# aperezhortal/pySPEEDY

Measured on AMD Instinct MI355X. Metric: simulated-years/day (whole node), T30L8, higher is better.
Workload: dtype f64

## Files before the change

### include/pyspeedy_amd.h

```cpp
#ifndef PYSPEEDY_AMD_H
#define PYSPEEDY_AMD_H

#include <stddef.h>
#include <stdint.h>

#ifdef __cplusplus
extern "C" {
#endif

#define SPD_IX 96
#define SPD_IL 48
#define SPD_IY 24
#define SPD_KX 8
#define SPD_MX 31
#define SPD_NX 32
#define SPD_TRUNC 30

#define SPD_OK 0
#define SPD_E_ARG (-1)
#define SPD_E_DEVICE (-2)
#define SPD_E_SIZE (-3)
#define SPD_E_TIMEOUT (-4)

typedef struct spd_context *spd_handle;

int spd_create(spd_handle *out, int device);
int spd_destroy(spd_handle h);
int spd_device(spd_handle h);
const char *spd_last_error(void);
const char *spd_version(void);

long spd_get_table_host(spd_handle h, const char *name, double *buf_host, size_t buf_elems);

int spd_calendar_walk(int year, int month, int day, int hour, int minute, int nsteps, int32_t *ymdhm, int32_t *month_idx,
                      int32_t *imont1, double *tmonth, double *tyear);
int spd_daily_forcing_host(double tyear, double *out);

int spd_spec2grid(spd_handle h, const double *spec, double *grid, int kcos, int nfields, void *stream);
int spd_grid2spec(spd_handle h, const double *grid, double *spec, int nfields, void *stream);
int spd_legendre_inv(spd_handle h, const double *spec, double *four, int nfields, void *stream);
int spd_legendre(spd_handle h, const double *four, double *spec, int nfields, void *stream);
int spd_fourier_inv(spd_handle h, const double *four, double *grid, int kcos, int nfields, void *stream);
int spd_fourier(spd_handle h, const double *grid, double *four, int nfields, void *stream);

int spd_vort2vel(spd_handle h, const double *vor, const double *div, double *ucos, double *vcos, int nfields,
                 void *stream);
int spd_vel2vort(spd_handle h, const double *ucos, const double *vcos, double *vor, double *div, int nfields,
                 void *stream);
int spd_grid_vel2vort(spd_handle h, const double *ug, const double *vg, double *vor, double *div, int kcos,
                      int nfields, void *stream);
int spd_gradient(spd_handle h, const double *psi, double *psdx, double *psdy, int nfields, void *stream);
int spd_laplacian(spd_handle h, const double *in, double *out, int inverse, int nfields, void *stream);
int spd_truncate(spd_handle h, double *field, int nfields, void *stream);
int spd_grid_filter(spd_handle h, const double *fg1, double *fg2, int nfields, void *stream);

typedef struct spd_physics_args {
    const double *ug, *vg, *tg, *qg, *phig;
    const double *pslg;
    double *utend, *vtend, *ttend, *qtend;
    const double *fmask_land, *phis0, *forog, *sst_am, *alb_land, *alb_sea, *snowc, *land_temp, *soil_avail_water;
    const double *flux_solar_in, *flux_ozone_upper, *flux_ozone_lower, *zenit_correction, *stratospheric_correction,
        *alb_surface;
    double *precnv, *precls, *cbmf, *slrd, *slr, *olr;
    double *slru, *ustr, *vstr, *shf, *evap, *hfluxn;
    double *rad_st4a;
    double *rad_flux;
    double *tt_rsw;
    double *rad_tau2;
    double *rad_strat_corr;
    double *tsr, *ssrd, *ssr, *qcloud_equiv;
    int32_t *iptop, *icltop;
    double *ts, *tskin, *u0, *v0, *t0, *cloudc, *clstr;
// ... 125 lines not shown
```

### pyspeedy_amd/_lib.py

```python
import ctypes as C
import os
import subprocess

_HERE = os.path.dirname(os.path.abspath(__file__))
LIB_PATH = os.environ.get("PYSPEEDY_AMD_LIB") or os.path.join(_HERE, "libpyspeedy_amd.so")
CSRC = os.path.join(_HERE, "csrc")

IX, IL, IY, KX, MX, NX, TRUNC = 96, 48, 24, 8, 31, 32, 30
NSPEC, NFOUR, NGRID = MX * NX, 2 * MX * IL, IX * IL

SPD_OK, SPD_E_ARG, SPD_E_DEVICE, SPD_E_SIZE = 0, -1, -2, -3
SPD_STATS_MEAN, SPD_STATS_VARIANCE, SPD_STATS_STD = 0, 1, 2


class SpeedyHipError(RuntimeError):
    pass


def build(verbose=False):
    cmd = ["make", "-C", CSRC, "-j4"]
    if not verbose:
        cmd.insert(1, "-s")
    subprocess.run(cmd, check=True)
    if not os.path.isfile(LIB_PATH):
# ... 16 lines not shown
    _fields_ = [(n, C.c_void_p) for n in _PHYS_PTR_FIELDS] + [
        ("air_absortivity_co2", C.c_double), ("compute_shortwave", C.c_int32), ("fp32", C.c_int32),
        ("sppt_pattern", C.c_void_p)]


class ModelControl(C.Structure):
    _fields_ = [(n, C.c_int32) for n in (
        "current_step", "year", "month", "day", "hour", "minute", "month_idx", "land_coupling_flag",
        "sst_anomaly_coupling_flag", "increase_co2", "sppt_on", "sppt_first", "physics_fp32", "reserved")] + [
        ("sppt_step", C.c_int64), ("sppt_first_member_id", C.c_int64), ("sppt_seed", C.c_uint64),
        ("air_absortivity_co2", C.c_double), ("ablco2_ref", C.c_double)]


class StreamProbeArgs(C.Structure):
    _fields_ = [(n, C.c_int32) for n in (
        "reads", "writes", "lane_bytes", "in_flight", "nontemporal", "waves_per_simd", "rows_per_wave", "reps", "layout",
        "reserved")] + [
        ("total_bytes", C.c_uint64)]


_SIGNATURES = {
    "spd_stream_probe": (C.c_int, [C.c_void_p, C.POINTER(StreamProbeArgs), C.POINTER(C.c_double), C.POINTER(C.c_double),
                                   C.POINTER(C.c_uint64), C.POINTER(C.c_uint64)]),
    "spd_create": (C.c_int, [C.POINTER(C.c_void_p), C.c_int]),
    "spd_destroy": (C.c_int, [C.c_void_p]),
    "spd_device": (C.c_int, [C.c_void_p]),
    "spd_last_error": (C.c_char_p, []),
    "spd_version": (C.c_char_p, []),
    "spd_get_table_host": (C.c_long, [C.c_void_p, C.c_char_p, C.c_void_p, C.c_size_t]),
    "spd_calendar_walk": (C.c_int, [C.c_int] * 6 + [C.c_void_p] * 5),
    "spd_daily_forcing_host": (C.c_int, [C.c_double, C.c_void_p]),
    "spd_spec2grid": (C.c_int, [C.c_void_p, C.c_void_p, C.c_void_p, C.c_int, C.c_int, C.c_void_p]),
    "spd_grid2spec": (C.c_int, [C.c_void_p, C.c_void_p, C.c_void_p, C.c_int, C.c_void_p]),
    "spd_legendre_inv": (C.c_int, [C.c_void_p, C.c_void_p, C.c_void_p, C.c_int, C.c_void_p]),
    "spd_legendre": (C.c_int, [C.c_void_p, C.c_void_p, C.c_void_p, C.c_int, C.c_void_p]),
    "spd_fourier_inv": (C.c_int, [C.c_void_p, C.c_void_p, C.c_void_p, C.c_int, C.c_int, C.c_void_p]),
    "spd_fourier": (C.c_int, [C.c_void_p, C.c_void_p, C.c_void_p, C.c_int, C.c_void_p]),
    "spd_vort2vel": (C.c_int, [C.c_void_p] + [C.c_void_p] * 4 + [C.c_int, C.c_void_p]),
    "spd_vel2vort": (C.c_int, [C.c_void_p] + [C.c_void_p] * 4 + [C.c_int, C.c_void_p]),
    "spd_grid_vel2vort": (C.c_int, [C.c_void_p] + [C.c_void_p] * 4 + [C.c_int, C.c_int, C.c_void_p]),
    "spd_gradient": (C.c_int, [C.c_void_p] + [C.c_void_p] * 3 + [C.c_int, C.c_void_p]),
    "spd_laplacian": (C.c_int, [C.c_void_p, C.c_void_p, C.c_void_p, C.c_int, C.c_int, C.c_void_p]),
    "spd_truncate": (C.c_int, [C.c_void_p, C.c_void_p, C.c_int, C.c_void_p]),
    "spd_grid_filter": (C.c_int, [C.c_void_p, C.c_void_p, C.c_void_p, C.c_int, C.c_void_p]),
    "spd_physics": (C.c_int, [C.c_void_p, C.POINTER(PhysicsArgs), C.c_int, C.c_void_p]),
    "spd_model_create": (C.c_int, [C.c_void_p, C.c_int, C.POINTER(C.c_void_p)]),
    "spd_model_destroy": (C.c_int, [C.c_void_p]),
    "spd_model_members": (C.c_int, [C.c_void_p]),
    "spd_model_memory": (C.c_int, [C.c_void_p, C.POINTER(C.c_size_t), C.POINTER(C.c_size_t)]),
    "spd_model_var_bytes": (C.c_long, [C.c_void_p, C.c_char_p]),
    "spd_model_var_storage": (C.c_int, [C.c_void_p, C.c_char_p]),
    "spd_model_set": (C.c_int, [C.c_void_p, C.c_char_p, C.c_int, C.c_void_p, C.c_size_t]),
    "spd_model_get": (C.c_int, [C.c_void_p, C.c_char_p, C.c_int, C.c_void_p, C.c_size_t]),
    "spd_model_device_ptr": (C.c_void_p, [C.c_void_p, C.c_char_p]),
    "spd_model_invalidate": (C.c_int, [C.c_void_p]),
    "spd_model_checks_in_flight": (C.c_int, [C.c_void_p]),
    "spd_model_set_co2": (C.c_int, [C.c_void_p, C.c_double]),
    "spd_model_co2": (C.c_double, [C.c_void_p]),
    "spd_model_set_time_step": (C.c_int, [C.c_void_p, C.c_double]),
    "spd_model_step_dynamics": (C.c_int, [C.c_void_p, C.c_int, C.c_int, C.c_double, C.c_int, C.c_void_p]),
    "spd_model_check": (C.c_int, [C.c_void_p, C.c_int, C.c_void_p, C.c_void_p, C.c_void_p]),
    "spd_model_check_begin": (C.c_int, [C.c_void_p, C.c_int, C.c_void_p]),
    "spd_model_check_end": (C.c_int, [C.c_void_p, C.c_int, C.c_void_p]),
    "spd_model_check_defer": (C.c_int, [C.c_void_p, C.c_int, C.c_void_p]),
    "spd_model_check_settle": (C.c_int, [C.c_void_p, C.c_int]),
    "spd_model_check_counts": (C.c_int, [C.c_void_p, C.POINTER(C.c_int32), C.POINTER(C.c_int32)]),
# ... 113 lines not shown
```

### pyspeedy_amd/csrc/capi.hip

```cpp
#include <hip/hip_runtime.h>

#include <cstdio>
#include <cstring>
#include <mutex>
#include <string>
#include <vector>

#include "../../include/pyspeedy_amd.h"
#include "context.hpp"
#include "device_tables.hpp"
#include "surface_host.hpp"
#include "vertical_consts.hpp"

namespace spd {
hipError_t run_spec2grid(const DeviceTables &T, int stage, const double *src, double *dst, int kcos, int nfields,
                         hipStream_t stream);
hipError_t run_grid2spec(const DeviceTables &T, int stage, const double *src, double *dst, int prescale, int nfields,
                         hipStream_t stream);
hipError_t run_vort2vel(const DeviceTables &T, const double *vor, const double *div, double *ucos, double *vcos,
                        int nfields, hipStream_t s);
hipError_t run_vel2vort(const DeviceTables &T, const double *ucos, const double *vcos, double *vor, double *div,
                        int nfields, hipStream_t s);
hipError_t run_gradient(const DeviceTables &T, const double *psi, double *psdx, double *psdy, int nfields, hipStream_t s);
hipError_t run_scale(const double *in, double *out, const double *table, double sign, int nfields, hipStream_t s);
hipError_t run_physics(const DeviceTables &T, const spd_physics_args &a, int nmembers, int fp32, hipStream_t s);
}

using namespace spd;

static thread_local std::string g_last_error;

static int fail(int code, const std::string &msg) {
    g_last_error = msg;
    return code;
}

int spd_set_error(int code, const std::string &msg) { return fail(code, msg); }

static int hip_fail(hipError_t e, const char *what) {
    return fail(SPD_E_DEVICE, std::string(what) + ": " + hipGetErrorString(e));
}

#define SPD_HIP(call)                                  \
    do {                                               \
        hipError_t e_ = (call);                        \
        if (e_ != hipSuccess) {                        \
            (void)hipGetLastError();  \
            return hip_fail(e_, #call);                \
        }                                              \
    } while (0)

// ... 250 lines not shown
    return SPD_OK;
}

static int done(hipError_t e, const char *fn) { return e == hipSuccess ? SPD_OK : hip_fail(e, fn); }

static int get_scratch(spd_handle h, size_t bytes, double **out) {
    std::lock_guard<std::mutex> lock(h->scratch_mutex);
    if (bytes > h->scratch_bytes) {
        SPD_HIP(hipDeviceSynchronize());
        if (h->scratch) SPD_HIP(hipFree(h->scratch));
        h->scratch = nullptr;
        h->scratch_bytes = 0;
        void *p = nullptr;
        SPD_HIP(hipMalloc(&p, bytes));
        h->scratch = static_cast<double *>(p);
        h->scratch_bytes = bytes;
    }
    *out = h->scratch;
    return SPD_OK;
}

extern "C" {

int spd_spec2grid(spd_handle h, const double *spec, double *grid, int kcos, int nfields, void *stream) {
    if (int rc = check(h, nfields, "spd_spec2grid", {spec, grid})) return rc;
    return done(run_spec2grid(h->dev, 0, spec, grid, kcos, nfields, static_cast<hipStream_t>(stream)), "spd_spec2grid");
}

int spd_grid2spec(spd_handle h, const double *grid, double *spec, int nfields, void *stream) {
    if (int rc = check(h, nfields, "spd_grid2spec", {grid, spec})) return rc;
    return done(run_grid2spec(h->dev, 0, grid, spec, 0, nfields, static_cast<hipStream_t>(stream)), "spd_grid2spec");
}

int spd_legendre_inv(spd_handle h, const double *spec, double *four, int nfields, void *stream) {
    if (int rc = check(h, nfields, "spd_legendre_inv", {spec, four})) return rc;
    return done(run_spec2grid(h->dev, 1, spec, four, 1, nfields, static_cast<hipStream_t>(stream)), "spd_legendre_inv");
}

int spd_legendre(spd_handle h, const double *four, double *spec, int nfields, void *stream) {
    if (int rc = check(h, nfields, "spd_legendre", {four, spec})) return rc;
    return done(run_grid2spec(h->dev, 1, four, spec, 0, nfields, static_cast<hipStream_t>(stream)), "spd_legendre");
}

int spd_fourier_inv(spd_handle h, const double *four, double *grid, int kcos, int nfields, void *stream) {
    if (int rc = check(h, nfields, "spd_fourier_inv", {four, grid})) return rc;
    return done(run_spec2grid(h->dev, 2, four, grid, kcos, nfields, static_cast<hipStream_t>(stream)), "spd_fourier_inv");
}

int spd_fourier(spd_handle h, const double *grid, double *four, int nfields, void *stream) {
    if (int rc = check(h, nfields, "spd_fourier", {grid, four})) return rc;
    return done(run_grid2spec(h->dev, 2, grid, four, 0, nfields, static_cast<hipStream_t>(stream)), "spd_fourier");
}

int spd_vort2vel(spd_handle h, const double *vor, const double *div, double *ucos, double *vcos, int nfields, void *stream) {
    if (int rc = check(h, nfields, "spd_vort2vel", {vor, div, ucos, vcos})) return rc;
    return done(run_vort2vel(h->dev, vor, div, ucos, vcos, nfields, static_cast<hipStream_t>(stream)), "spd_vort2vel");
}

int spd_vel2vort(spd_handle h, const double *ucos, const double *vcos, double *vor, double *div, int nfields, void *stream) {
    if (int rc = check(h, nfields, "spd_vel2vort", {ucos, vcos, vor, div})) return rc;
    return done(run_vel2vort(h->dev, ucos, vcos, vor, div, nfields, static_cast<hipStream_t>(stream)), "spd_vel2vort");
}

int spd_grid_vel2vort(spd_handle h, const double *ug, const double *vg, double *vor, double *div, int kcos, int nfields,
                      void *stream) {
    if (int rc = check(h, nfields, "spd_grid_vel2vort", {ug, vg, vor, div})) return rc;
// ... 63 lines not shown
```

### pyspeedy_amd/csrc/fft96.hpp

```cpp
#pragma once
#include <hip/hip_runtime.h>

namespace spd {
namespace fft {

__device__ constexpr double kTaur = -0.5;
__device__ constexpr double kTaui = 0.866025388240814209;
__device__ constexpr double kSqrt2 = 1.414213538169860840;
__device__ constexpr double kHsqt2 = 0.707106769084930420;
constexpr int kNumGroups = 7;
constexpr int kNumBlocks = 8;
constexpr int kInvLast = 60;

struct Pair { double r, i; };

template <bool ZeroPad>
__device__ inline void radb2_pair(const double *in, const double *W, int i1, Pair &h1, Pair &h2) {
    const double ar = in[i1 - 2], ai = in[i1 - 1];
    const int q = 96 - i1;
    double br = in[q], bi = in[q + 1];
    if (ZeroPad) {
        br = (q > kInvLast) ? 0.0 : br;
        bi = (q + 1 > kInvLast) ? 0.0 : bi;
    }
// ... 330 lines not shown
#pragma unroll
        for (int i = 0; i < 3; ++i) x[j][i] = in[12 * kk + 3 * j + i];
    double y[4][3];
    {
        const double tr1 = x[0][0] - x[3][2], tr2 = x[0][0] + x[3][2];
        const double tr3 = x[1][2] + x[1][2], tr4 = x[2][0] + x[2][0];
        y[0][0] = tr2 + tr3; y[1][0] = tr1 - tr4; y[2][0] = tr2 - tr3; y[3][0] = tr1 + tr4;
    }
    {
        const double ti1 = x[0][2] + x[3][1], ti2 = x[0][2] - x[3][1], ti3 = x[2][2] - x[1][1], tr4 = x[2][2] + x[1][1];
        const double tr1 = x[0][1] - x[3][0], tr2 = x[0][1] + x[3][0], ti4 = x[2][1] - x[1][0], tr3 = x[2][1] + x[1][0];
        const double cr3 = tr2 - tr3, ci3 = ti2 - ti3;
        const double cr2 = tr1 - tr4, cr4 = tr1 + tr4, ci2 = ti1 + ti4, ci4 = ti1 - ti4;
        y[0][1] = tr2 + tr3;
        y[0][2] = ti2 + ti3;
        y[1][1] = W[84] * cr2 - W[85] * ci2;
        y[1][2] = W[84] * ci2 + W[85] * cr2;
        y[2][1] = W[87] * cr3 - W[88] * ci3;
        y[2][2] = W[87] * ci3 + W[88] * cr3;
        y[3][1] = W[90] * cr4 - W[91] * ci4;
        y[3][2] = W[90] * ci4 + W[91] * cr4;
    }
#pragma unroll
    for (int j = 0; j < 4; ++j) {
        const double tr2 = y[j][1] + y[j][1];
        const double cr2 = y[j][0] + kTaur * tr2;
        const double ci3 = kTaui * (y[j][2] + y[j][2]);
        o[j][0] = y[j][0] + tr2;
        o[j][1] = cr2 - ci3;
        o[j][2] = cr2 + ci3;
    }
}

__device__ inline void fwd_block_r(const double *in, const double *W, int kk, double (&o)[12]) {
    double y[4][3];
#pragma unroll
    for (int j = 0; j < 4; ++j) {
        const double *c = in + kk + 8 * j;
        const double c1 = c[0], c2 = c[32], c3 = c[64];
        const double cr2 = c2 + c3;
        y[j][0] = c1 + cr2;
        y[j][2] = kTaui * (c3 - c2);
        y[j][1] = c1 + kTaur * cr2;
    }
    {
        const double tr1 = y[1][0] + y[3][0], tr2 = y[0][0] + y[2][0];
        o[0] = tr1 + tr2;
        o[11] = tr2 - tr1;
        o[5] = y[0][0] - y[2][0];
        o[6] = y[3][0] - y[1][0];
    }
    {
        const double cr2 = W[84] * y[1][1] + W[85] * y[1][2], ci2 = W[84] * y[1][2] - W[85] * y[1][1];
        const double cr3 = W[87] * y[2][1] + W[88] * y[2][2], ci3 = W[87] * y[2][2] - W[88] * y[2][1];
        const double cr4 = W[90] * y[3][1] + W[91] * y[3][2], ci4 = W[90] * y[3][2] - W[91] * y[3][1];
        const double tr1 = cr2 + cr4, tr4 = cr4 - cr2, ti1 = ci2 + ci4, ti4 = ci2 - ci4;
        const double ti2 = y[0][2] + ci3, ti3 = y[0][2] - ci3, tr2 = y[0][1] + cr3, tr3 = y[0][1] - cr3;
        o[1] = tr1 + tr2; o[9] = tr2 - tr1; o[2] = ti1 + ti2; o[10] = ti1 - ti2;
        o[7] = ti4 + tr3; o[3] = tr3 - ti4; o[8] = tr4 + ti3; o[4] = tr4 - ti3;
    }
}

struct Quad { double lo_r, lo_i, hi_r, hi_i; };

__device__ inline Quad radf2_pair_r(const Pair &h1, const Pair &h2, const double *W, int i1, double scale) {
    const double wr = W[i1 - 3], wi = W[i1 - 2];
    const double tr2 = wr * h2.r + wi * h2.i;
    const double ti2 = wr * h2.i - wi * h2.r;
    Quad q;
    q.lo_i = (h1.i + ti2) * scale;
    q.lo_r = (h1.r + tr2) * scale;
    q.hi_i = (ti2 - h1.i) * scale;
    q.hi_r = (h1.r - tr2) * scale;
    return q;
}

__device__ inline void fwd_group_general_r(const double *in, const double *W, int i, double scale, Quad (&q)[4]) {
    const double w1r = W[48 + i - 3], w1i = W[48 + i - 2];
    const double w2r = W[60 + i - 3], w2i = W[60 + i - 2];
    const double w3r = W[72 + i - 3], w3i = W[72 + i - 2];
    Pair a[2], b[2], c[2], d[2];
#pragma unroll
    for (int k = 0; k < 2; ++k) {
        const double *x = in + (i - 2) + 12 * k;
        const double x1r = x[0], x1i = x[1], x2r = x[24], x2i = x[25], x3r = x[48], x3i = x[49], x4r = x[72], x4i = x[73];
        const double cr2 = w1r * x2r + w1i * x2i, ci2 = w1r * x2i - w1i * x2r;
        const double cr3 = w2r * x3r + w2i * x3i, ci3 = w2r * x3i - w2i * x3r;
        const double cr4 = w3r * x4r + w3i * x4i, ci4 = w3r * x4i - w3i * x4r;
        const double tr1 = cr2 + cr4, tr4 = cr4 - cr2, ti1 = ci2 + ci4, ti4 = ci2 - ci4;
        const double ti2 = x1i + ci3, ti3 = x1i - ci3, tr2 = x1r + cr3, tr3 = x1r - cr3;
        a[k].r = tr1 + tr2;  a[k].i = ti1 + ti2;
        d[k].r = tr2 - tr1;  d[k].i = ti1 - ti2;
        c[k].r = ti4 + tr3;  c[k].i = tr4 + ti3;
        b[k].r = tr3 - ti4;  b[k].i = tr4 - ti3;
    }
    q[0] = radf2_pair_r(a[0], a[1], W, i, scale);
    q[1] = radf2_pair_r(b[0], b[1], W, 26 - i, scale);
    q[2] = radf2_pair_r(c[0], c[1], W, i + 24, scale);
    q[3] = radf2_pair_r(d[0], d[1], W, 50 - i, scale);
}

__device__ inline void fwd_group_general_store(double *row, int i, const Quad (&q)[4]) {
    row[i - 2] = q[0].lo_r;       row[i - 1] = q[0].lo_i;
    row[24 - i] = q[1].lo_r;      row[25 - i] = q[1].lo_i;
    row[i + 22] = q[2].lo_r;      row[i + 23] = q[2].lo_i;
    row[48 - i] = q[3].lo_r;      row[49 - i] = q[3].lo_i;
    row[46 + i] = q[3].hi_r;      row[47 + i] = q[3].hi_i;
}

__device__ inline void fwd_group_first_r(const double *in, const double *W, double scale, double (&o)[5]) {
    double p0[2], p47[2];
    Pair m[2];
#pragma unroll
    for (int k = 0; k < 2; ++k) {
        const double *x = in + 12 * k;
        const double tr1 = x[24] + x[72], tr2 = x[0] + x[48];
        p0[k] = tr1 + tr2;
        p47[k] = tr2 - tr1;
        m[k].r = x[0] - x[48];
        m[k].i = x[72] - x[24];
    }
    o[0] = (p0[0] + p0[1]) * scale;
    o[1] = p47[0] * scale;
    o[2] = (-p47[1]) * scale;
    const Quad q = radf2_pair_r(m[0], m[1], W, 25, scale);
    o[3] = q.lo_r;
    o[4] = q.lo_i;
}

__device__ inline void fwd_group_last_r(const double *in, const double *W, double scale, Quad (&q)[4]) {
    Pair a[2], b[2];
#pragma unroll
    for (int k = 0; k < 2; ++k) {
        const double *x = in + 11 + 12 * k;
        const double ti1 = -kHsqt2 * (x[24] + x[72]);
        const double tr1 = kHsqt2 * (x[24] - x[72]);
        a[k].r = tr1 + x[0];
        b[k].r = x[0] - tr1;
        a[k].i = ti1 - x[48];
        b[k].i = ti1 + x[48];
    }
    q[0] = radf2_pair_r(a[0], a[1], W, 13, scale);
    q[1] = radf2_pair_r(b[0], b[1], W, 37, scale);
}

}
}
```

### pyspeedy_amd/csrc/transforms.hip

```cpp
#include <hip/hip_runtime.h>

#include "device_tables.hpp"
#include "diagnostics_block.hpp"
#include "launch_events.hpp"
#include "fft96.hpp"

namespace spd {

constexpr int kThreads = 512;
constexpr int kRowStride = 97;
constexpr int kRows = IL;
constexpr int kCStride = 63;
constexpr int kCBufDoubles = kRows * kCStride;
constexpr int kSpecPerLane = (NSPEC + kThreads - 1) / kThreads;
constexpr int kGridPerLane = (NGRID / 2 + kThreads - 1) / kThreads;
constexpr int kPlanePerLane = (kRows * MX + kThreads - 1) / kThreads;
constexpr int kHalfPlanePerLane = (IY * MX + kThreads - 1) / kThreads;
constexpr int kInvLanes = MX * 12;
constexpr size_t kLdsBytes = (kCBufDoubles + 2 * NSPEC) * sizeof(double);
static_assert(kRows * kRowStride <= kCBufDoubles + 2 * NSPEC, "R must fit inside C + S");

enum class Stage { Fused, LegendreOnly, FourierOnly };

using d2 = double __attribute__((ext_vector_type(2)));
// ... 175 lines not shown

    const bool as_float = (kcos & kGridAsFloat) != 0;
    kcos &= ~kGridAsFloat;
    gd2_out g = (gd2_out)dst;
    double cs[kGridPerLane];
#pragma unroll
    for (int it = 0; it < kGridPerLane; ++it) {
        const int idx = tid + it * kThreads;
        cs[it] = (kcos != 1 && idx < NGRID / 2) ? T.cosgr[idx / (IX / 2)] : 1.0;
    }
#pragma unroll
    for (int it = 0; it < kGridPerLane; ++it) {
        const int idx = tid + it * kThreads;
        if (idx < NGRID / 2) {
            const int r = idx / (IX / 2), ip = idx - r * (IX / 2);
            const double *a = rows + r * kRowStride + 2 * ip;
            d2 v{a[0], a[1]};
            if (kcos != 1) {
                v.x *= cs[it];
                v.y *= cs[it];
            }
            if (as_float) {
                const f2 w{static_cast<float>(v.x), static_cast<float>(v.y)};
                __builtin_nontemporal_store(w, &((gf2_out)dst)[idx]);
                continue;
            }
            __builtin_nontemporal_store(v, &g[idx]);
        }
    }
    TRACE_MARK(0, 4);
    TRACE_END(0);
}

template <Stage ST>
__device__ __forceinline__ void grid2spec_body(const double *__restrict__ src, double *__restrict__ dst,
                                               const DeviceTables &T, int prescale) {
    extern __shared__ __attribute__((aligned(16))) double lds[];
    double *rows = lds;
    double *cbuf = lds;
    d2 *s = reinterpret_cast<d2 *>(lds + kCBufDoubles);
    const int tid = threadIdx.x;
    const int wave = wave_id(), lane = tid & 63;

    TRACE_BEGIN();
    if (ST == Stage::Fused) {
        gd2_in g = (gd2_in)src;
        constexpr int kPairTasks = IY * (IX / 2);
        constexpr int kPairPerLane = (kPairTasks + kThreads - 1) / kThreads;
        d2 gn[kPairPerLane], gs[kPairPerLane];
        double wj[kPairPerLane], cn[kPairPerLane], cs[kPairPerLane];
        const double *ctab = (prescale == 1) ? T.cosgr : T.cosgr2;
#pragma unroll
        for (int it = 0; it < kPairPerLane; ++it) {
            const int idx = tid + it * kThreads;
            if (idx < kPairTasks) {
                const int j = idx / (IX / 2), ip = idx - j * (IX / 2);
                gn[it] = __builtin_nontemporal_load(&g[(kRows - 1 - j) * (IX / 2) + ip]);
                gs[it] = __builtin_nontemporal_load(&g[j * (IX / 2) + ip]);
                wj[it] = T.wt[j];
                cn[it] = (prescale != 0) ? ctab[kRows - 1 - j] : 1.0;
                cs[it] = (prescale != 0) ? ctab[j] : 1.0;
            }
        }
#pragma unroll
        for (int it = 0; it < kPairPerLane; ++it) {
            const int idx = tid + it * kThreads;
            if (idx < kPairTasks) {
                const int j = idx / (IX / 2), ip = idx - j * (IX / 2);
                d2 n = gn[it], so = gs[it];
                if (prescale != 0) {
                    n.x *= cn[it];
                    n.y *= cn[it];
                    so.x *= cs[it];
                    so.y *= cs[it];
                }
                const double w = wj[it];
                double *an = rows + (kRows - 1 - j) * kRowStride + 2 * ip, *as = rows + j * kRowStride + 2 * ip;
                an[0] = (n.x + so.x) * w;
                an[1] = (n.y + so.y) * w;
                as[0] = (n.x - so.x) * w;
                as[1] = (n.y - so.y) * w;
            }
        }
    } else if (ST == Stage::FourierOnly) {
        gd2_in g = (gd2_in)src;
        d2 gv[kGridPerLane];
        double cs[kGridPerLane];
        const double *ctab = (prescale == 1) ? T.cosgr : T.cosgr2;
#pragma unroll
        for (int it = 0; it < kGridPerLane; ++it) {
            const int idx = tid + it * kThreads;
            if (idx < NGRID / 2) gv[it] = __builtin_nontemporal_load(&g[idx]);
            cs[it] = (prescale != 0 && idx < NGRID / 2) ? ctab[idx / (IX / 2)] : 1.0;
        }
#pragma unroll
        for (int it = 0; it < kGridPerLane; ++it) {
            const int idx = tid + it * kThreads;
            if (idx < NGRID / 2) {
                const int r = idx / (IX / 2), ip = idx - r * (IX / 2);
                d2 v = gv[it];
                if (prescale != 0) {
                    v.x *= cs[it];
                    v.y *= cs[it];
                }
                double *a = rows + r * kRowStride + 2 * ip;
                a[0] = v.x;
                a[1] = v.y;
            }
        }
    }
    if (ST != Stage::LegendreOnly) {
        __syncthreads();
        TRACE_MARK(1, 0);
        double *row = rows + lane * kRowStride;
        const bool active = lane < kRows;
        {
            double o[12];
            if (active) fft::fwd_block_r(row, T.work, wave, o);
            __syncthreads();
            if (active) {
#pragma unroll
                for (int e = 0; e < 12; ++e) row[12 * wave + e] = o[e];
            }
        }
        __syncthreads();
        TRACE_MARK(1, 1);
        {
            fft::Quad q[4];
            double o5[5];
            if (active && wave < fft::kNumGroups) {
                if (wave < 5)
                    fft::fwd_group_general_r(row, T.work, 3 + 2 * wave, T.fft_scale, q);
                else if (wave == 5)
                    fft::fwd_group_first_r(row, T.work, T.fft_scale, o5);
                else
                    fft::fwd_group_last_r(row, T.work, T.fft_scale, q);
            }
            __syncthreads();
            if (ST == Stage::Fused)
                for (int idx = tid; idx < NSPEC; idx += kThreads) s[idx] = d2{0.0, 0.0};
            double *crow = cbuf + lane * kCStride;
            if (active && wave < fft::kNumGroups) {
                if (wave < 5) {
                    fft::fwd_group_general_store(crow, 3 + 2 * wave, q);
                } else if (wave == 5) {
                    crow[0] = o5[0]; crow[47] = o5[1]; crow[48] = o5[2]; crow[23] = o5[3]; crow[24] = o5[4];
                    crow[61] = 0.0;
                } else {
                    crow[11] = q[0].lo_r; crow[12] = q[0].lo_i;
                    crow[35] = q[1].lo_r; crow[36] = q[1].lo_i;
                    crow[59] = q[1].hi_r; crow[60] = q[1].hi_i;
                }
            }
        }
        __syncthreads();
        TRACE_MARK(1, 2);
    } else {
        gd2_in g = (gd2_in)src;
        d2 nv[kHalfPlanePerLane], sv[kHalfPlanePerLane];
        double w[kHalfPlanePerLane];
#pragma unroll
        for (int it = 0; it < kHalfPlanePerLane; ++it) {
            const int item = tid + it * kThreads;
            if (item < IY * MX) {
                const int j = item / MX, m = item - j * MX;
                nv[it] = g[(kRows - 1 - j) * MX + m];
                sv[it] = g[j * MX + m];
                w[it] = T.wt[j];
            }
        }
        for (int idx = tid; idx < NSPEC; idx += kThreads) s[idx] = d2{0.0, 0.0};
#pragma unroll
        for (int it = 0; it < kHalfPlanePerLane; ++it) {
            const int item = tid + it * kThreads;
            if (item < IY * MX) {
                const int j = item / MX, m = item - j * MX;
                const int pr = pos_re(m), pi = pos_im(m);
                double *rn = cbuf + (kRows - 1 - j) * kCStride, *rs = cbuf + j * kCStride;
                rn[pr] = (nv[it].x + sv[it].x) * w[it];
                rs[pr] = (nv[it].x - sv[it].x) * w[it];
                rn[pi] = (nv[it].y + sv[it].y) * w[it];
                rs[pi] = (nv[it].y - sv[it].y) * w[it];
            }
        }
        __syncthreads();
    }

// ... 4 lines not shown
            g[idx] = (r == 1) ? 0.0 : cbuf[r0 * kCStride + (r == 0 ? 0 : r - 1)];
        }
        return;
    }

    TRACE_MARK(1, 3);
    if (tid < T.ndir) {
        const int4 meta = reinterpret_cast<const int4 *>(T.dirmeta)[tid];
        const int pr = meta.x & 0xff, pi = meta.x >> 8, par = meta.y;
        double acc[2][2] = {{0.0, 0.0}, {0.0, 0.0}};
        const d2 *pol = reinterpret_cast<const d2 *>(T.pdir) + tid;
        const int pstride = T.dir_stride;
        const double *base = cbuf + (par ? 0 : (kRows - 1) * kCStride);
        const int rstep = par ? kCStride : -kCStride;
#pragma unroll 4
        for (int j = 0; j < IY; ++j) {
            const d2 p = pol[j * pstride];
            const double *r = base + j * rstep;
            const double xr = r[pr], xi = r[pi];
            acc[0][0] += p.x * xr;  acc[0][1] += p.x * xi;
            acc[1][0] += p.y * xr;  acc[1][1] += p.y * xi;
        }
        s[meta.z] = d2{acc[0][0], acc[0][1]};
        if (meta.w >= 0) s[meta.w] = d2{acc[1][0], acc[1][1]};
    }
    __syncthreads();
    TRACE_MARK(1, 4);
    gd2_out g = (gd2_out)dst;
    for (int idx = tid; idx < NSPEC; idx += kThreads) __builtin_nontemporal_store(s[idx], &g[idx]);
    TRACE_MARK(1, 5);
    TRACE_END(1);
}

template <Stage ST>
__global__ __launch_bounds__(kThreads) void spec2grid_kernel(const double *__restrict__ src, double *__restrict__ dst,
                                                             DeviceTables T, int kcos) {
    const size_t f = blockIdx.x;
    constexpr size_t in = (ST == Stage::FourierOnly) ? NFOUR : 2 * NSPEC, out = (ST == Stage::LegendreOnly) ? NFOUR : NGRID;
    spec2grid_body<ST>(src + f * in, dst + f * out, T, kcos);
}

template <Stage ST>
__global__ __launch_bounds__(kThreads) void grid2spec_kernel(const double *__restrict__ src, double *__restrict__ dst,
                                                             DeviceTables T, int prescale) {
    const size_t f = blockIdx.x;
    constexpr size_t in = (ST == Stage::LegendreOnly) ? NFOUR : NGRID, out = (ST == Stage::FourierOnly) ? NFOUR : 2 * NSPEC;
    grid2spec_body<ST>(src + f * in, dst + f * out, T, prescale);
}

__global__ __launch_bounds__(kThreads) void spec2grid_table_kernel(const FieldDesc *__restrict__ table, DeviceTables T) {
    const FieldDesc e = table[blockIdx.x];
    spec2grid_body<Stage::Fused>(e.src, e.dst, T, e.flag, e.mode, e.src2);
}

static_assert(kThreads == 64 * KX, "a check block is a workgroup of the transform launch");
__global__ __launch_bounds__(kThreads, 8) void spec2grid_table_check_kernel(const FieldDesc *__restrict__ table, DeviceTables T,
                                                                            int members, CheckArgs check) {
    const int front = (members + 7) & ~7;
    if (static_cast<int>(blockIdx.x) < front) {
        if (static_cast<int>(blockIdx.x) < members) diagnostics_block<2>(check, T, check.first + static_cast<int>(blockIdx.x));
        return;
    }
    const FieldDesc e = table[blockIdx.x - front];
    spec2grid_body<Stage::Fused>(e.src, e.dst, T, e.flag, e.mode, e.src2);
}

__global__ __launch_bounds__(kThreads) void grid2spec_table_kernel(const FieldDesc *__restrict__ table, DeviceTables T) {
    const FieldDesc e = table[blockIdx.x];
    grid2spec_body<Stage::Fused>(e.src, e.dst, T, e.flag);
}

static hipError_t configure_once(const void *kernel, bool (&done)[64]) {
    int dev = 0;
    if (hipGetDevice(&dev) != hipSuccess || dev < 0 || dev >= 64) return hipErrorInvalidDevice;
    if (done[dev]) return hipSuccess;
    const hipError_t e = hipFuncSetAttribute(kernel, hipFuncAttributeMaxDynamicSharedMemorySize, static_cast<int>(kLdsBytes));
    done[dev] = e == hipSuccess;
    return e;
}
#define SPD_CONFIGURE(kernel)                                            \
    ([] {                                                                \
        static bool done[64] = {};                                       \
        return configure_once(reinterpret_cast<const void *>(kernel), done); \
    }())

template <Stage ST>
static hipError_t launch_s2g(const double *src, double *dst, const DeviceTables &T, int nfields, int kcos, hipStream_t st) {
    const hipError_t cfg = SPD_CONFIGURE(&spec2grid_kernel<ST>);
    if (cfg != hipSuccess) return cfg;
    hipLaunchKernelGGL((spec2grid_kernel<ST>), dim3(nfields), dim3(kThreads), kLdsBytes, st, src, dst, T, kcos);
    return hipGetLastError();
}

template <Stage ST>
static hipError_t launch_g2s(const double *src, double *dst, const DeviceTables &T, int nfields, int prescale,
                             hipStream_t st) {
    const hipError_t cfg = SPD_CONFIGURE(&grid2spec_kernel<ST>);
    if (cfg != hipSuccess) return cfg;
    hipLaunchKernelGGL((grid2spec_kernel<ST>), dim3(nfields), dim3(kThreads), kLdsBytes, st, src, dst, T, prescale);
    return hipGetLastError();
}

hipError_t run_spec2grid_table(const DeviceTables &T, const FieldDesc *table, int nfields, hipStream_t st) {
    if (nfields == 0) return hipSuccess;
    const hipError_t cfg = SPD_CONFIGURE(&spec2grid_table_kernel);
    if (cfg != hipSuccess) return cfg;
    launch(spec2grid_table_kernel, dim3(nfields), dim3(kThreads), kLdsBytes, st, table, T);
    return hipGetLastError();
}

hipError_t run_spec2grid_table_check(const DeviceTables &T, const FieldDesc *table, int nfields, const CheckArgs &check, int members,
                                     hipStream_t st) {
    const hipError_t cfg = SPD_CONFIGURE(&spec2grid_table_check_kernel);
    if (cfg != hipSuccess) return cfg;
    launch(spec2grid_table_check_kernel, dim3(((members + 7) & ~7) + nfields), dim3(kThreads), kLdsBytes, st, table, T, members, check);
    return hipGetLastError();
}

hipError_t run_grid2spec_table(const DeviceTables &T, const FieldDesc *table, int nfields, hipStream_t st) {
    if (nfields == 0) return hipSuccess;
    const hipError_t cfg = SPD_CONFIGURE(&grid2spec_table_kernel);
    if (cfg != hipSuccess) return cfg;
    launch(grid2spec_table_kernel, dim3(nfields), dim3(kThreads), kLdsBytes, st, table, T);
    return hipGetLastError();
}

hipError_t run_spec2grid(const DeviceTables &T, int stage, const double *src, double *dst, int kcos, int nfields,
                         hipStream_t stream) {
    if (nfields == 0) return hipSuccess;
    switch (stage) {
        case 0: return launch_s2g<Stage::Fused>(src, dst, T, nfields, kcos, stream);
        case 1: return launch_s2g<Stage::LegendreOnly>(src, dst, T, nfields, kcos, stream);
        default: return launch_s2g<Stage::FourierOnly>(src, dst, T, nfields, kcos, stream);
    }
}

hipError_t run_grid2spec(const DeviceTables &T, int stage, const double *src, double *dst, int prescale, int nfields,
                         hipStream_t stream) {
    if (nfields == 0) return hipSuccess;
    switch (stage) {
        case 0: return launch_g2s<Stage::Fused>(src, dst, T, nfields, prescale, stream);
        case 1: return launch_g2s<Stage::LegendreOnly>(src, dst, T, nfields, prescale, stream);
        default: return launch_g2s<Stage::FourierOnly>(src, dst, T, nfields, prescale, stream);
    }
}

}

#ifdef SPD_TRACE
extern "C" int spd_trace_read(double *out , double *count ) {
    unsigned long long acc[2][8], cnt[2], zero[2][8] = {};
    if (hipMemcpyFromSymbol(acc, HIP_SYMBOL(spd::spd_trace_acc), sizeof(acc)) != hipSuccess) return -1;
    if (hipMemcpyFromSymbol(cnt, HIP_SYMBOL(spd::spd_trace_cnt), sizeof(cnt)) != hipSuccess) return -1;
    for (int d = 0; d < 2; ++d) {
        count[d] = static_cast<double>(cnt[d]);
        for (int i = 0; i < 8; ++i) out[d * 8 + i] = cnt[d] ? static_cast<double>(acc[d][i]) / cnt[d] : 0.0;
// ... 7 lines not shown
```

Before: 1.693 million.

## Process two fields per block in grid-to-spectral table kernel with shared Legendre pass

The table-driven grid-to-spectral kernel now handles two fields per workgroup. The second field's grid load is issued early to overlap the first field's FFT. The first field's Fourier coefficients are parked in registers and then moved to a second LDS plane. A single Legendre pass then reads each polynomial value once for both fields. Fewer blocks are launched, and launch bounds plus a larger LDS allocation are set. This amortizes table reads and hides load latency, at the cost of more registers and LDS per block, and possibly lower occupancy. A new C API entry for testing the table path is also added.

Result: no change. 1.685 million (-0.5%).

```diff
diff --git a/include/pyspeedy_amd.h b/include/pyspeedy_amd.h
--- a/include/pyspeedy_amd.h
+++ b/include/pyspeedy_amd.h
@@ -38,6 +38,8 @@
 
 int spd_spec2grid(spd_handle h, const double *spec, double *grid, int kcos, int nfields, void *stream);
 int spd_grid2spec(spd_handle h, const double *grid, double *spec, int nfields, void *stream);
+int spd_grid2spec_table(spd_handle h, const double *grid, double *spec, const int32_t *prescale_host, int nfields, int first,
+                        void *stream);
 int spd_legendre_inv(spd_handle h, const double *spec, double *four, int nfields, void *stream);
 int spd_legendre(spd_handle h, const double *four, double *spec, int nfields, void *stream);
 int spd_fourier_inv(spd_handle h, const double *four, double *grid, int kcos, int nfields, void *stream);
diff --git a/pyspeedy_amd/_lib.py b/pyspeedy_amd/_lib.py
--- a/pyspeedy_amd/_lib.py
+++ b/pyspeedy_amd/_lib.py
@@ -72,6 +72,7 @@
     "spd_daily_forcing_host": (C.c_int, [C.c_double, C.c_void_p]),
     "spd_spec2grid": (C.c_int, [C.c_void_p, C.c_void_p, C.c_void_p, C.c_int, C.c_int, C.c_void_p]),
     "spd_grid2spec": (C.c_int, [C.c_void_p, C.c_void_p, C.c_void_p, C.c_int, C.c_void_p]),
+    "spd_grid2spec_table": (C.c_int, [C.c_void_p, C.c_void_p, C.c_void_p, C.c_void_p, C.c_int, C.c_int, C.c_void_p]),
     "spd_legendre_inv": (C.c_int, [C.c_void_p, C.c_void_p, C.c_void_p, C.c_int, C.c_void_p]),
     "spd_legendre": (C.c_int, [C.c_void_p, C.c_void_p, C.c_void_p, C.c_int, C.c_void_p]),
     "spd_fourier_inv": (C.c_int, [C.c_void_p, C.c_void_p, C.c_void_p, C.c_int, C.c_int, C.c_void_p]),
diff --git a/pyspeedy_amd/csrc/capi.hip b/pyspeedy_amd/csrc/capi.hip
--- a/pyspeedy_amd/csrc/capi.hip
+++ b/pyspeedy_amd/csrc/capi.hip
@@ -17,6 +17,7 @@
                          hipStream_t stream);
 hipError_t run_grid2spec(const DeviceTables &T, int stage, const double *src, double *dst, int prescale, int nfields,
                          hipStream_t stream);
+hipError_t run_grid2spec_table(const DeviceTables &T, const FieldDesc *table, int nfields, hipStream_t st);
 hipError_t run_vort2vel(const DeviceTables &T, const double *vor, const double *div, double *ucos, double *vcos,
                         int nfields, hipStream_t s);
 hipError_t run_vel2vort(const DeviceTables &T, const double *ucos, const double *vcos, double *vor, double *div,
@@ -333,6 +334,27 @@
     return done(run_grid2spec(h->dev, 0, grid, spec, 0, nfields, static_cast<hipStream_t>(stream)), "spd_grid2spec");
 }
 
+int spd_grid2spec_table(spd_handle h, const double *grid, double *spec, const int32_t *prescale_host, int nfields, int first,
+                        void *stream) {
+    if (int rc = check(h, nfields, "spd_grid2spec_table", {grid, spec, prescale_host})) return rc;
+    if (first < 0 || first > nfields) return fail(SPD_E_ARG, "spd_grid2spec_table: first outside [0, nfields]");
+    if (first == nfields) return SPD_OK;
+    std::vector<FieldDesc> host(static_cast<size_t>(nfields));
+    for (int i = 0; i < nfields; ++i) {
+        if (prescale_host[i] < 0 || prescale_host[i] > 2) return fail(SPD_E_ARG, "spd_grid2spec_table: prescale outside 0..2");
+        host[i] = FieldDesc{grid + static_cast<size_t>(i) * NGRID, spec + static_cast<size_t>(i) * 2 * NSPEC, prescale_host[i], 0, nullptr};
+    }
+    SPD_HIP(hipSetDevice(h->device));
+    void *table = nullptr;
+    SPD_HIP(hipMalloc(&table, host.size() * sizeof(FieldDesc)));
+    hipStream_t s = static_cast<hipStream_t>(stream);
+    hipError_t e = hipMemcpy(table, host.data(), host.size() * sizeof(FieldDesc), hipMemcpyHostToDevice);
+    if (e == hipSuccess) e = run_grid2spec_table(h->dev, static_cast<const FieldDesc *>(table) + first, nfields - first, s);
+    if (e == hipSuccess) e = hipStreamSynchronize(s);
+    (void)hipFree(table);
+    return done(e, "spd_grid2spec_table");
+}
+
 int spd_legendre_inv(spd_handle h, const double *spec, double *four, int nfields, void *stream) {
     if (int rc = check(h, nfields, "spd_legendre_inv", {spec, four})) return rc;
     return done(run_spec2grid(h->dev, 1, spec, four, 1, nfields, static_cast<hipStream_t>(stream)), "spd_legendre_inv");
diff --git a/pyspeedy_amd/csrc/fft96.hpp b/pyspeedy_amd/csrc/fft96.hpp
--- a/pyspeedy_amd/csrc/fft96.hpp
+++ b/pyspeedy_amd/csrc/fft96.hpp
@@ -386,7 +386,8 @@
     }
 }
 
-__device__ inline void fwd_block_r(const double *in, const double *W, int kk, double (&o)[12]) {
+template <class WP>
+__device__ inline void fwd_block_r(const double *in, WP W, int kk, double (&o)[12]) {
     double y[4][3];
 #pragma unroll
     for (int j = 0; j < 4; ++j) {
@@ -417,7 +418,8 @@
 
 struct Quad { double lo_r, lo_i, hi_r, hi_i; };
 
-__device__ inline Quad radf2_pair_r(const Pair &h1, const Pair &h2, const double *W, int i1, double scale) {
+template <class WP>
+__device__ inline Quad radf2_pair_r(const Pair &h1, const Pair &h2, WP W, int i1, double scale) {
     const double wr = W[i1 - 3], wi = W[i1 - 2];
     const double tr2 = wr * h2.r + wi * h2.i;
     const double ti2 = wr * h2.i - wi * h2.r;
@@ -429,7 +431,8 @@
     return q;
 }
 
-__device__ inline void fwd_group_general_r(const double *in, const double *W, int i, double scale, Quad (&q)[4]) {
+template <class WP>
+__device__ inline void fwd_group_general_r(const double *in, WP W, int i, double scale, Quad (&q)[4]) {
     const double w1r = W[48 + i - 3], w1i = W[48 + i - 2];
     const double w2r = W[60 + i - 3], w2i = W[60 + i - 2];
     const double w3r = W[72 + i - 3], w3i = W[72 + i - 2];
@@ -462,7 +465,8 @@
     row[46 + i] = q[3].hi_r;      row[47 + i] = q[3].hi_i;
 }
 
-__device__ inline void fwd_group_first_r(const double *in, const double *W, double scale, double (&o)[5]) {
+template <class WP>
+__device__ inline void fwd_group_first_r(const double *in, WP W, double scale, double (&o)[5]) {
     double p0[2], p47[2];
     Pair m[2];
 #pragma unroll
@@ -482,7 +486,8 @@
     o[4] = q.lo_i;
 }
 
-__device__ inline void fwd_group_last_r(const double *in, const double *W, double scale, Quad (&q)[4]) {
+template <class WP>
+__device__ inline void fwd_group_last_r(const double *in, WP W, double scale, Quad (&q)[4]) {
     Pair a[2], b[2];
 #pragma unroll
     for (int k = 0; k < 2; ++k) {
diff --git a/pyspeedy_amd/csrc/transforms.hip b/pyspeedy_amd/csrc/transforms.hip
--- a/pyspeedy_amd/csrc/transforms.hip
+++ b/pyspeedy_amd/csrc/transforms.hip
@@ -231,6 +231,109 @@
     TRACE_END(0);
 }
 
+constexpr int kPairTasks = IY * (IX / 2);
+constexpr int kPairPerLane = (kPairTasks + kThreads - 1) / kThreads;
+
+struct GridStage {
+    d2 gn[kPairPerLane], gs[kPairPerLane];
+    double wj[kPairPerLane], cn[kPairPerLane], cs[kPairPerLane];
+};
+
+__device__ __forceinline__ void g2s_load_grid(const double *__restrict__ src, int tid, GridStage &r) {
+    gd2_in g = (gd2_in)src;
+#pragma unroll
+    for (int it = 0; it < kPairPerLane; ++it) {
+        const int idx = tid + it * kThreads;
+        if (idx < kPairTasks) {
+            const int j = idx / (IX / 2), ip = idx - j * (IX / 2);
+            r.gn[it] = __builtin_nontemporal_load(&g[(kRows - 1 - j) * (IX / 2) + ip]);
+            r.gs[it] = __builtin_nontemporal_load(&g[j * (IX / 2) + ip]);
+        }
+    }
+}
+
+__device__ __forceinline__ void g2s_load_factors(const DeviceTables &T, int prescale, int tid, GridStage &r) {
+    const double *ctab = (prescale == 1) ? T.cosgr : T.cosgr2;
+#pragma unroll
+    for (int it = 0; it < kPairPerLane; ++it) {
+        const int idx = tid + it * kThreads;
+        if (idx < kPairTasks) {
+            const int j = idx / (IX / 2);
+            r.wj[it] = T.wt[j];
+            r.cn[it] = (prescale != 0) ? ctab[kRows - 1 - j] : 1.0;
+            r.cs[it] = (prescale != 0) ? ctab[j] : 1.0;
+        }
+    }
+}
+
+__device__ __forceinline__ void g2s_store_grid(double *rows, int prescale, int tid, const GridStage &r) {
+#pragma unroll
+    for (int it = 0; it < kPairPerLane; ++it) {
+        const int idx = tid + it * kThreads;
+        if (idx < kPairTasks) {
+            const int j = idx / (IX / 2), ip = idx - j * (IX / 2);
+            d2 n = r.gn[it], so = r.gs[it];
+            if (prescale != 0) {
+                n.x *= r.cn[it];
+                n.y *= r.cn[it];
+                so.x *= r.cs[it];
+                so.y *= r.cs[it];
+            }
+            const double w = r.wj[it];
+            double *an = rows + (kRows - 1 - j) * kRowStride + 2 * ip, *as = rows + j * kRowStride + 2 * ip;
+            an[0] = (n.x + so.x) * w;
+            an[1] = (n.y + so.y) * w;
+            as[0] = (n.x - so.x) * w;
+            as[1] = (n.y - so.y) * w;
+        }
+    }
+}
+
+template <class WP>
+__device__ __forceinline__ void g2s_fft_block(double *rows, WP work, int wave, int lane) {
+    double *row = rows + lane * kRowStride;
+    const bool active = lane < kRows;
+    double o[12];
+    if (active) fft::fwd_block_r(row, work, wave, o);
+    __syncthreads();
+    if (active) {
+#pragma unroll
+        for (int e = 0; e < 12; ++e) row[12 * wave + e] = o[e];
+    }
+}
+
+template <class WP>
+__device__ __forceinline__ void g2s_fft_group(double *rows, WP work, double fft_scale, int wave, int lane, d2 *zero_s) {
+    double *row = rows + lane * kRowStride;
+    const bool active = lane < kRows;
+    fft::Quad q[4];
+    double o5[5];
+    if (active && wave < fft::kNumGroups) {
+        if (wave < 5)
+            fft::fwd_group_general_r(row, work, 3 + 2 * wave, fft_scale, q);
+        else if (wave == 5)
+            fft::fwd_group_first_r(row, work, fft_scale, o5);
+        else
+            fft::fwd_group_last_r(row, work, fft_scale, q);
+    }
+    __syncthreads();
+    if (zero_s)
+        for (int idx = threadIdx.x; idx < NSPEC; idx += kThreads) zero_s[idx] = d2{0.0, 0.0};
+    double *crow = rows + lane * kCStride;
+    if (active && wave < fft::kNumGroups) {
+        if (wave < 5) {
+            fft::fwd_group_general_store(crow, 3 + 2 * wave, q);
+        } else if (wave == 5) {
+            crow[0] = o5[0]; crow[47] = o5[1]; crow[48] = o5[2]; crow[23] = o5[3]; crow[24] = o5[4];
+            crow[61] = 0.0;
+        } else {
+            crow[11] = q[0].lo_r; crow[12] = q[0].lo_i;
+            crow[35] = q[1].lo_r; crow[36] = q[1].lo_i;
+            crow[59] = q[1].hi_r; crow[60] = q[1].hi_i;
+        }
+    }
+}
+
 template <Stage ST>
 __device__ __forceinline__ void grid2spec_body(const double *__restrict__ src, double *__restrict__ dst,
                                                const DeviceTables &T, int prescale) {
@@ -243,44 +346,10 @@
 
     TRACE_BEGIN();
     if (ST == Stage::Fused) {
-        gd2_in g = (gd2_in)src;
-        constexpr int kPairTasks = IY * (IX / 2);
-        constexpr int kPairPerLane = (kPairTasks + kThreads - 1) / kThreads;
-        d2 gn[kPairPerLane], gs[kPairPerLane];
-        double wj[kPairPerLane], cn[kPairPerLane], cs[kPairPerLane];
-        const double *ctab = (prescale == 1) ? T.cosgr : T.cosgr2;
-#pragma unroll
-        for (int it = 0; it < kPairPerLane; ++it) {
-            const int idx = tid + it * kThreads;
-            if (idx < kPairTasks) {
-                const int j = idx / (IX / 2), ip = idx - j * (IX / 2);
-                gn[it] = __builtin_nontemporal_load(&g[(kRows - 1 - j) * (IX / 2) + ip]);
-                gs[it] = __builtin_nontemporal_load(&g[j * (IX / 2) + ip]);
-                wj[it] = T.wt[j];
-                cn[it] = (prescale != 0) ? ctab[kRows - 1 - j] : 1.0;
-                cs[it] = (prescale != 0) ? ctab[j] : 1.0;
-            }
-        }
-#pragma unroll
-        for (int it = 0; it < kPairPerLane; ++it) {
-            const int idx = tid + it * kThreads;
-            if (idx < kPairTasks) {
-                const int j = idx / (IX / 2), ip = idx - j * (IX / 2);
-                d2 n = gn[it], so = gs[it];
-                if (prescale != 0) {
-                    n.x *= cn[it];
-                    n.y *= cn[it];
-                    so.x *= cs[it];
-                    so.y *= cs[it];
-                }
-                const double w = wj[it];
-                double *an = rows + (kRows - 1 - j) * kRowStride + 2 * ip, *as = rows + j * kRowStride + 2 * ip;
-                an[0] = (n.x + so.x) * w;
-                an[1] = (n.y + so.y) * w;
-                as[0] = (n.x - so.x) * w;
-                as[1] = (n.y - so.y) * w;
-            }
-        }
+        GridStage r;
+        g2s_load_grid(src, tid, r);
+        g2s_load_factors(T, prescale, tid, r);
+        g2s_store_grid(rows, prescale, tid, r);
     } else if (ST == Stage::FourierOnly) {
         gd2_in g = (gd2_in)src;
         d2 gv[kGridPerLane];
@@ -311,47 +380,10 @@
     if (ST != Stage::LegendreOnly) {
         __syncthreads();
         TRACE_MARK(1, 0);
-        double *row = rows + lane * kRowStride;
-        const bool active = lane < kRows;
-        {
-            double o[12];
-            if (active) fft::fwd_block_r(row, T.work, wave, o);
-            __syncthreads();
-            if (active) {
-#pragma unroll
-                for (int e = 0; e < 12; ++e) row[12 * wave + e] = o[e];
-            }
-        }
+        g2s_fft_block(rows, T.work, wave, lane);
         __syncthreads();
         TRACE_MARK(1, 1);
-        {
-            fft::Quad q[4];
-            double o5[5];
-            if (active && wave < fft::kNumGroups) {
-                if (wave < 5)
-                    fft::fwd_group_general_r(row, T.work, 3 + 2 * wave, T.fft_scale, q);
-                else if (wave == 5)
-                    fft::fwd_group_first_r(row, T.work, T.fft_scale, o5);
-                else
-                    fft::fwd_group_last_r(row, T.work, T.fft_scale, q);
-            }
-            __syncthreads();
-            if (ST == Stage::Fused)
-                for (int idx = tid; idx < NSPEC; idx += kThreads) s[idx] = d2{0.0, 0.0};
-            double *crow = cbuf + lane * kCStride;
-            if (active && wave < fft::kNumGroups) {
-                if (wave < 5) {
-                    fft::fwd_group_general_store(crow, 3 + 2 * wave, q);
-                } else if (wave == 5) {
-                    crow[0] = o5[0]; crow[47] = o5[1]; crow[48] = o5[2]; crow[23] = o5[3]; crow[24] = o5[4];
-                    crow[61] = 0.0;
-                } else {
-                    crow[11] = q[0].lo_r; crow[12] = q[0].lo_i;
-                    crow[35] = q[1].lo_r; crow[36] = q[1].lo_i;
-                    crow[59] = q[1].hi_r; crow[60] = q[1].hi_i;
-                }
-            }
-        }
+        g2s_fft_group(rows, T.work, T.fft_scale, wave, lane, ST == Stage::Fused ? s : nullptr);
         __syncthreads();
         TRACE_MARK(1, 2);
     } else {
@@ -422,6 +454,111 @@
     TRACE_END(1);
 }
 
+constexpr size_t kPairLdsBytes = 2 * kCBufDoubles * sizeof(double);
+constexpr int kCPerLane = (kCBufDoubles + kThreads - 1) / kThreads;
+static_assert(static_cast<size_t>(kRows * kRowStride) * sizeof(double) <= kPairLdsBytes, "R must fit inside the two planes");
+static_assert(4 * NSPEC * sizeof(double) <= kPairLdsBytes, "both output staging areas must fit inside the two planes");
+
+__device__ __forceinline__ void grid2spec_pair_body(const FieldDesc &ea, const FieldDesc &eb, const DeviceTables &T) {
+    extern __shared__ __attribute__((aligned(16))) double lds[];
+    double *rows = lds;
+    double *cb = lds;
+    double *ca = lds + kCBufDoubles;
+    d2 *sa = reinterpret_cast<d2 *>(lds);
+    d2 *sb = sa + NSPEC;
+    const int tid = threadIdx.x;
+    const int wave = wave_id(), lane = tid & 63;
+
+    const auto work = (const __attribute__((address_space(4))) double *)T.work;
+    TRACE_BEGIN();
+    GridStage r, rb;
+    g2s_load_grid(ea.src, tid, r);
+    g2s_load_factors(T, ea.flag, tid, r);
+    g2s_store_grid(rows, ea.flag, tid, r);
+    int tid_b = tid;
+    asm volatile("" : "+v"(tid_b));
+    __builtin_assume(tid_b >= 0 && tid_b < kThreads);
+    g2s_load_grid(eb.src, tid_b, rb);
+    __syncthreads();
+    TRACE_MARK(1, 0);
+    g2s_fft_block(rows, work, wave, lane);
+    __syncthreads();
+    g2s_fft_group(rows, work, T.fft_scale, wave, lane, nullptr);
+    __syncthreads();
+    double keep[kCPerLane];
+#pragma unroll
+    for (int it = 0; it < kCPerLane; ++it)
+        if (tid + it * kThreads < kCBufDoubles) keep[it] = cb[tid + it * kThreads];
+    int tid_s = tid;
+    asm volatile("" : "+v"(tid_s));
+    __builtin_assume(tid_s >= 0 && tid_s < kThreads);
+    g2s_load_factors(T, eb.flag, tid_s, rb);
+    __syncthreads();
+    TRACE_MARK(1, 1);
+    g2s_store_grid(rows, eb.flag, tid_s, rb);
+    __syncthreads();
+    TRACE_MARK(1, 2);
+    g2s_fft_block(rows, work, wave, lane);
+    __syncthreads();
+    g2s_fft_group(rows, work, T.fft_scale, wave, lane, nullptr);
+#pragma unroll
+    for (int it = 0; it < kCPerLane; ++it)
+        if (tid + it * kThreads < kCBufDoubles) ca[tid + it * kThreads] = keep[it];
+    __syncthreads();
+    TRACE_MARK(1, 3);
+
+    const bool owner = tid < T.ndir;
+    int4 meta = int4{0, 0, 0, -1};
+    double acc[2][2][2] = {{{0.0, 0.0}, {0.0, 0.0}}, {{0.0, 0.0}, {0.0, 0.0}}};
+    if (owner) {
+        meta = reinterpret_cast<const int4 *>(T.dirmeta)[tid];
+        const int pr = meta.x & 0xff, pi = meta.x >> 8, par = meta.y;
+        const d2 *pol = reinterpret_cast<const d2 *>(T.pdir) + tid;
+        const int pstride = T.dir_stride;
+        const int first = par ? 0 : (kRows - 1) * kCStride;
+        const int rstep = par ? kCStride : -kCStride;
+#pragma unroll 4
+        for (int j = 0; j < IY; ++j) {
+            const d2 p = pol[j * pstride];
+            const double *xa = ca + first + j * rstep, *xb = cb + first + j * rstep;
+            const double ar = xa[pr], ai = xa[pi], br = xb[pr], bi = xb[pi];
+            acc[0][0][0] += p.x * ar;  acc[0][0][1] += p.x * ai;
+            acc[0][1][0] += p.y * ar;  acc[0][1][1] += p.y * ai;
+            acc[1][0][0] += p.x * br;  acc[1][0][1] += p.x * bi;
+            acc[1][1][0] += p.y * br;  acc[1][1][1] += p.y * bi;
+        }
+    }
+    __syncthreads();
+    for (int idx = tid; idx < 2 * NSPEC; idx += kThreads) sa[idx] = d2{0.0, 0.0};
+    __syncthreads();
+    if (owner) {
+        sa[meta.z] = d2{acc[0][0][0], acc[0][0][1]};
+        sb[meta.z] = d2{acc[1][0][0], acc[1][0][1]};
+        if (meta.w >= 0) {
+            sa[meta.w] = d2{acc[0][1][0], acc[0][1][1]};
+            sb[meta.w] = d2{acc[1][1][0], acc[1][1][1]};
+        }
+    }
+    __syncthreads();
+    TRACE_MARK(1, 4);
+    gd2_out ga = (gd2_out)ea.dst, gb = (gd2_out)eb.dst;
+    d2 va[kSpecPerLane], vb[kSpecPerLane];
+#pragma unroll
+    for (int it = 0; it < kSpecPerLane; ++it)
+        if (tid + it * kThreads < NSPEC) {
+            va[it] = sa[tid + it * kThreads];
+            vb[it] = sb[tid + it * kThreads];
+        }
+#pragma unroll
+    for (int it = 0; it < kSpecPerLane; ++it)
+        if (tid + it * kThreads < NSPEC) {
+            __builtin_nontemporal_store(va[it], &ga[tid + it * kThreads]);
+            __builtin_nontemporal_store(vb[it], &gb[tid + it * kThreads]);
+        }
+    TRACE_MARK(1, 5);
+    TRACE_END(1);
+}
+
 template <Stage ST>
 __global__ __launch_bounds__(kThreads) void spec2grid_kernel(const double *__restrict__ src, double *__restrict__ dst,
                                                              DeviceTables T, int kcos) {
@@ -455,28 +592,34 @@
     spec2grid_body<Stage::Fused>(e.src, e.dst, T, e.flag, e.mode, e.src2);
 }
 
-__global__ __launch_bounds__(kThreads) void grid2spec_table_kernel(const FieldDesc *__restrict__ table, DeviceTables T) {
-    const FieldDesc e = table[blockIdx.x];
-    grid2spec_body<Stage::Fused>(e.src, e.dst, T, e.flag);
-}
-
-static hipError_t configure_once(const void *kernel, bool (&done)[64]) {
+__global__ __launch_bounds__(kThreads, 6) void grid2spec_table_kernel(const FieldDesc *__restrict__ table, DeviceTables T,
+                                                                      int nfields) {
+    const int first = 2 * static_cast<int>(blockIdx.x);
+    if (first + 1 < nfields) {
+        grid2spec_pair_body(table[first], table[first + 1], T);
+    } else {
+        const FieldDesc e = table[first];
+        grid2spec_body<Stage::Fused>(e.src, e.dst, T, e.flag);
+    }
+}
+
+static hipError_t configure_once(const void *kernel, bool (&done)[64], size_t bytes) {
     int dev = 0;
     if (hipGetDevice(&dev) != hipSuccess || dev < 0 || dev >= 64) return hipErrorInvalidDevice;
     if (done[dev]) return hipSuccess;
-    const hipError_t e = hipFuncSetAttribute(kernel, hipFuncAttributeMaxDynamicSharedMemorySize, static_cast<int>(kLdsBytes));
+    const hipError_t e = hipFuncSetAttribute(kernel, hipFuncAttributeMaxDynamicSharedMemorySize, static_cast<int>(bytes));
     done[dev] = e == hipSuccess;
     return e;
 }
-#define SPD_CONFIGURE(kernel)                                            \
-    ([] {                                                                \
-        static bool done[64] = {};                                       \
-        return configure_once(reinterpret_cast<const void *>(kernel), done); \
+#define SPD_CONFIGURE(kernel, bytes)                                               \
+    ([] {                                                                          \
+        static bool done[64] = {};                                                 \
+        return configure_once(reinterpret_cast<const void *>(kernel), done, bytes); \
     }())
 
 template <Stage ST>
 static hipError_t launch_s2g(const double *src, double *dst, const DeviceTables &T, int nfields, int kcos, hipStream_t st) {
-    const hipError_t cfg = SPD_CONFIGURE(&spec2grid_kernel<ST>);
+    const hipError_t cfg = SPD_CONFIGURE(&spec2grid_kernel<ST>, kLdsBytes);
     if (cfg != hipSuccess) return cfg;
     hipLaunchKernelGGL((spec2grid_kernel<ST>), dim3(nfields), dim3(kThreads), kLdsBytes, st, src, dst, T, kcos);
     return hipGetLastError();
@@ -485,7 +628,7 @@
 template <Stage ST>
 static hipError_t launch_g2s(const double *src, double *dst, const DeviceTables &T, int nfields, int prescale,
                              hipStream_t st) {
-    const hipError_t cfg = SPD_CONFIGURE(&grid2spec_kernel<ST>);
+    const hipError_t cfg = SPD_CONFIGURE(&grid2spec_kernel<ST>, kLdsBytes);
     if (cfg != hipSuccess) return cfg;
     hipLaunchKernelGGL((grid2spec_kernel<ST>), dim3(nfields), dim3(kThreads), kLdsBytes, st, src, dst, T, prescale);
     return hipGetLastError();
@@ -493,7 +636,7 @@
 
 hipError_t run_spec2grid_table(const DeviceTables &T, const FieldDesc *table, int nfields, hipStream_t st) {
     if (nfields == 0) return hipSuccess;
-    const hipError_t cfg = SPD_CONFIGURE(&spec2grid_table_kernel);
+    const hipError_t cfg = SPD_CONFIGURE(&spec2grid_table_kernel, kLdsBytes);
     if (cfg != hipSuccess) return cfg;
     launch(spec2grid_table_kernel, dim3(nfields), dim3(kThreads), kLdsBytes, st, table, T);
     return hipGetLastError();
@@ -501,7 +644,7 @@
 
 hipError_t run_spec2grid_table_check(const DeviceTables &T, const FieldDesc *table, int nfields, const CheckArgs &check, int members,
                                      hipStream_t st) {
-    const hipError_t cfg = SPD_CONFIGURE(&spec2grid_table_check_kernel);
+    const hipError_t cfg = SPD_CONFIGURE(&spec2grid_table_check_kernel, kLdsBytes);
     if (cfg != hipSuccess) return cfg;
     launch(spec2grid_table_check_kernel, dim3(((members + 7) & ~7) + nfields), dim3(kThreads), kLdsBytes, st, table, T, members, check);
     return hipGetLastError();
@@ -509,9 +652,9 @@
 
 hipError_t run_grid2spec_table(const DeviceTables &T, const FieldDesc *table, int nfields, hipStream_t st) {
     if (nfields == 0) return hipSuccess;
-    const hipError_t cfg = SPD_CONFIGURE(&grid2spec_table_kernel);
+    const hipError_t cfg = SPD_CONFIGURE(&grid2spec_table_kernel, kPairLdsBytes);
     if (cfg != hipSuccess) return cfg;
-    launch(grid2spec_table_kernel, dim3(nfields), dim3(kThreads), kLdsBytes, st, table, T);
+    launch(grid2spec_table_kernel, dim3((nfields + 1) / 2), dim3(kThreads), kPairLdsBytes, st, table, T, nfields);
     return hipGetLastError();
 }
 
```
